# ext-sakamoro/ALICE-Codec

Hardware: AMD Instinct MI355X
Metric: Mpixels/s encode+decode, 1080p x 64 CDF9/7 q=80; bit-exact vs CPU (higher is better)
Workload: dtype int32

## Files before the change

### alice-codec_amd/csrc/rans.hip

```cpp
#include <cstdlib>

#include "common.h"
#include "freq_table.h"
#include "kernels.h"

namespace alice {


__device__ inline RansEncEntry make_enc_entry(uint32_t f, uint32_t c) {
    RansEncEntry e;
    e.freq = f;
    e.cum = c;
    unsigned long long xm = (unsigned long long)f << 19;
    unsigned long long xm8 = (unsigned long long)f << 27;
    e.xmax = xm > 0xFFFFFFFFull ? 0xFFFFFFFFu : (uint32_t)xm;
    e.xmax8 = xm8 > 0xFFFFFFFFull ? 0xFFFFFFFFu : (uint32_t)xm8;
    if (f == 0u || f > kProbScale) {
        e.xmax = f == 0u ? 0xFFFFFFFFu : e.xmax;
        e.xmax8 = f == 0u ? 0xFFFFFFFFu : e.xmax8;
        e.rcp = 0u; e.rsh = 0u; e.g = 0; e.cbias = 0u;
    } else if (f == 1u) {
        e.rcp = 0xFFFFFFFFu; e.rsh = 0u; e.g = 4095; e.cbias = c + 4095u;
    } else {
        uint32_t L = 32u - (uint32_t)__clz((int)(f - 1u));
        unsigned long long p = 1ull << (31u + L);
        e.rcp = (uint32_t)((p + f - 1u) / f);
        e.rsh = L - 1u;
        e.g = (int32_t)kProbScale - (int32_t)f;
        e.cbias = c;
    }
    return e;
}

__device__ inline uint32_t build_dec_slots(uint32_t f, uint32_t c, uint32_t* scratch, RansDecSlots* __restrict__ out) {
    const int s = threadIdx.x;
    uint32_t end = c + f;
    if (end > kProbScale) end = kProbScale;
    __syncthreads();
    scratch[s] = c;
    scratch[256 + s] = c < end ? end : c;
    scratch[512 + s] = f;
    out->symtab[s] = (f & 0xFFFFu) | (c << 16);
    __syncthreads();
    uint32_t fl = 0u;
    for (uint32_t slot = (uint32_t)s; slot < kProbScale; slot += 256u) {
        uint32_t owner = 0u;
        for (uint32_t k = 0; k < 256u; ++k)
            if (slot >= scratch[k] && slot < scratch[256 + k]) owner = k;
        const uint32_t fo = scratch[512 + owner], co = scratch[owner];
        uint32_t fe, be;
        if (fo >= kProbScale) {
            fe = 0xFFFFFFFFu; be = (slot - co) - slot + 1u;
            fl |= fo > kProbScale ? kTableDecExact : kTableDecBig;
        } else {
            fe = fo << 20; be = (slot - co) - ((fo * slot) >> kProbBits);
        }
        out->ftab[slot] = fe;
        out->btab[slot] = be;
        out->c2s[slot] = (uint8_t)owner;
    }
    return fl;
}

__global__ __launch_bounds__(256) void rans_table_kernel(const uint32_t* __restrict__ hist,
                                                         RansTable* __restrict__ tables, uint32_t n_sym,
                                                         const uint32_t* __restrict__ used) {
    __shared__ uint32_t scratch[768];
    const int chain = blockIdx.x;
    const int s = threadIdx.x;
    const uint32_t count = (uint32_t)s < n_sym ? hist[(size_t)chain * 256 + s] : 0u;
    uint32_t f, c;
    freq_table_256(count, n_sym, scratch, f, c);
    tables[chain].enc[s] = make_enc_entry(f, c);
    uint32_t fl = build_dec_slots(f, c, scratch, &tables[chain].dec);
    const uint32_t occurs = used ? used[(size_t)chain * 256 + s] : count;
    if (occurs > 0u && f == 0u) fl |= kTableDiverges;
    if (occurs > 0u && f > kProbScale) fl |= kTableNeedsGeneric;
    __shared__ uint32_t flags_sh;
    if (s == 0) flags_sh = 0u;
    __syncthreads();
    if (fl) atomicOr(&flags_sh, fl);
    __syncthreads();
    if (s == 0) tables[chain].flags = flags_sh | kTableVerified;
}

__global__ __launch_bounds__(256) void rans_table_from_arrays_kernel(const uint16_t* __restrict__ cum,
                                                                     const uint16_t* __restrict__ freq,
                                                                     RansTable* __restrict__ table) {
    __shared__ uint32_t scratch[768];
    __shared__ uint32_t flags_sh;
    const int s = threadIdx.x;
    if (s == 0) flags_sh = 0u;
    table->enc[s] = make_enc_entry(freq[s], cum[s]);
    const uint32_t fl = build_dec_slots(freq[s], cum[s], scratch, &table->dec);
    if (fl) atomicOr(&flags_sh, fl);
    __syncthreads();
    if (s == 0) table->flags = flags_sh;
}

__device__ __forceinline__ void chain_take_turns(uint32_t enabled) {
    if (!enabled) return;
    const uint32_t turn = (uint32_t)(clock64() >> 17);
    const uint32_t slot = __builtin_amdgcn_s_getreg((3 << 11) | (0 << 6) | 4);
    if ((turn ^ slot) & 1u) __builtin_amdgcn_s_setprio(1);
    else __builtin_amdgcn_s_setprio(0);
}


constexpr int kEncTile = 1024;
constexpr int kEncTilePad = 128;

__device__ __forceinline__ void ripple64(uint32_t& xin, uint32_t& xout, uint32_t xmax, uint32_t xmax8,
                                         uint32_t rcp, uint32_t rsh, int32_t g, uint32_t cprev) {
    uint32_t k, y, q;
    unsigned long long m1;
#define ALICE_RIPPLE_STEP(TAIL)                                                     \
    "v_add_u32_dpp %[xin], %[xout], %[cprev] wave_shr:1 row_mask:0xf bank_mask:0xf\n\t" \
    "v_cmp_ge_u32_e64 %[m1], %[xin], %[xmax]\n\t"                                  \
    "v_cmp_ge_u32_e32 vcc, %[xin], %[xmax8]\n\t"                                   \
    "s_nop 0\n\t"                                                                    \
    "v_cndmask_b32_e64 %[k], 0, 8, %[m1]\n\t"                                      \
    "v_cndmask_b32_e64 %[k], %[k], 16, vcc\n\t"                                    \
    "v_lshrrev_b32_e32 %[y], %[k], %[xin]\n\t"                                     \
    "v_mul_hi_u32 %[q], %[y], %[rcp]\n\t"                                          \
    "v_lshrrev_b32_e32 %[q], %[rsh], %[q]\n\t"                                     \
    "v_mad_i32_i24 %[xout], %[q], %[g], %[y]\n\t" TAIL
#define ALICE_RIPPLE_STEP4 ALICE_RIPPLE_STEP("s_nop 1\n\t") ALICE_RIPPLE_STEP("s_nop 1\n\t") ALICE_RIPPLE_STEP("s_nop 1\n\t") ALICE_RIPPLE_STEP("s_nop 1\n\t")
#define ALICE_RIPPLE_STEP16 ALICE_RIPPLE_STEP4 ALICE_RIPPLE_STEP4 ALICE_RIPPLE_STEP4 ALICE_RIPPLE_STEP4
    asm volatile(
        "s_nop 1\n\t"
        ALICE_RIPPLE_STEP16 ALICE_RIPPLE_STEP16 ALICE_RIPPLE_STEP16 ALICE_RIPPLE_STEP16
        : [xin] "+v"(xin), [xout] "+v"(xout), [k] "=&v"(k), [y] "=&v"(y), [q] "=&v"(q), [m1] "=&s"(m1)
        : [xmax] "v"(xmax), [xmax8] "v"(xmax8), [rcp] "v"(rcp), [rsh] "v"(rsh), [g] "v"(g),
          [cprev] "v"(cprev)
        : "vcc");
#undef ALICE_RIPPLE_STEP16
#undef ALICE_RIPPLE_STEP4
#undef ALICE_RIPPLE_STEP
}

__device__ __forceinline__ void ripple64_clean(uint32_t& xin, uint32_t& xout, uint32_t thr, uint32_t k0, uint32_t k1,
                                               uint32_t rcp, uint32_t rsh, int32_t g, uint32_t cprev) {
    uint32_t k, y, q;
#define ALICE_RIPPLE_STEP                                                            \
    "v_add_u32_dpp %[xin], %[xout], %[cprev] wave_shr:1 row_mask:0xf bank_mask:0xf\n\t" \
    "v_cmp_ge_u32_e32 vcc, %[xin], %[thr]\n\t"                                     \
    "s_nop 1\n\t"                                                                  \
    "v_cndmask_b32_e32 %[k], %[k0], %[k1], vcc\n\t"                                \
    "v_lshrrev_b32_e32 %[y], %[k], %[xin]\n\t"                                     \
    "v_mul_hi_u32 %[q], %[y], %[rcp]\n\t"                                          \
    "v_lshrrev_b32_e32 %[q], %[rsh], %[q]\n\t"                                     \
    "v_mad_i32_i24 %[xout], %[q], %[g], %[y]\n\t"                                  \
    "s_nop 1\n\t"
#define ALICE_RIPPLE_STEP4 ALICE_RIPPLE_STEP ALICE_RIPPLE_STEP ALICE_RIPPLE_STEP ALICE_RIPPLE_STEP
#define ALICE_RIPPLE_STEP16 ALICE_RIPPLE_STEP4 ALICE_RIPPLE_STEP4 ALICE_RIPPLE_STEP4 ALICE_RIPPLE_STEP4
    asm volatile(
        "s_nop 1\n\t"
        ALICE_RIPPLE_STEP16 ALICE_RIPPLE_STEP16 ALICE_RIPPLE_STEP16 ALICE_RIPPLE_STEP16
        : [xin] "+v"(xin), [xout] "+v"(xout), [k] "=&v"(k), [y] "=&v"(y), [q] "=&v"(q)
        : [thr] "v"(thr), [k0] "v"(k0), [k1] "v"(k1), [rcp] "v"(rcp), [rsh] "v"(rsh), [g] "v"(g), [cprev] "v"(cprev)
        : "vcc");
#undef ALICE_RIPPLE_STEP16
#undef ALICE_RIPPLE_STEP4
#undef ALICE_RIPPLE_STEP
}

__device__ __forceinline__ void ripple64_comp(uint32_t& u, uint32_t& z, uint32_t kc, uint32_t tpp, uint32_t rcp, uint32_t rsh,
                                              int32_t g) {
    uint32_t m, q;
#define ALICE_RIPPLE_STEP                                                            \
    "v_add_u32_dpp %[u], %[z], %[kc] wave_shr:1 row_mask:0xf bank_mask:0xf\n\t"     \
    "v_mad_i64_i32 v[62:63], vcc, %[u], %[two24], v[60:61]\n\t"                    \
    "v_min_u32_e32 %[m], %[u], v63\n\t"                                           \
    "v_mul_hi_u32 %[q], %[m], %[rcp]\n\t"                                          \
    "v_lshrrev_b32_e32 %[q], %[rsh], %[q]\n\t"                                     \
    "v_mad_i32_i24 %[z], %[q], %[g], %[m]\n\t"                                     \
    "s_nop 1\n\t"
#define ALICE_RIPPLE_STEP4 ALICE_RIPPLE_STEP ALICE_RIPPLE_STEP ALICE_RIPPLE_STEP ALICE_RIPPLE_STEP
#define ALICE_RIPPLE_STEP16 ALICE_RIPPLE_STEP4 ALICE_RIPPLE_STEP4 ALICE_RIPPLE_STEP4 ALICE_RIPPLE_STEP4
    asm volatile(
        "v_mov_b32_e32 v60, 0\n\t"
        "v_mov_b32_e32 v61, %[tpp]\n\t"
        ALICE_RIPPLE_STEP16 ALICE_RIPPLE_STEP16 ALICE_RIPPLE_STEP16 ALICE_RIPPLE_STEP16
        : [u] "+v"(u), [z] "=&v"(z), [m] "=&v"(m), [q] "=&v"(q)
        : [kc] "v"(kc), [tpp] "v"(tpp), [rcp] "v"(rcp), [rsh] "v"(rsh), [g] "v"(g), [two24] "s"(1u << 24)
        : "v60", "v61", "v62", "v63", "vcc");
#undef ALICE_RIPPLE_STEP16
#undef ALICE_RIPPLE_STEP4
#undef ALICE_RIPPLE_STEP
}

template <bool kExclusive>
__global__ __launch_bounds__(64) void rans_encode_kernel(const uint8_t* __restrict__ sym_base,
                                                         unsigned long long sym_stride,
                                                         unsigned long long n_first,
                                                         const RansTable* __restrict__ tables,
                                                         uint8_t* __restrict__ out_base,
                                                         unsigned long long cap0,
                                                         unsigned long long group_stride,
                                                         unsigned long long group_head,
                                                         unsigned n_split,
                                                         RansResult* __restrict__ results,
                                                         unsigned long long cap1, unsigned long long cap2,
                                                         uint32_t x_init, uint32_t keep_open, uint32_t take_turns,
                                                         const RansEncodeDesc* __restrict__ descs) {
    __shared__ uint4 tab_a[256];
    __shared__ uint4 tab_b[256];
    __shared__ uint2 tab_c[256];
    __shared__ __attribute__((aligned(16))) uint8_t tile[kEncTilePad + kEncTile];

    if constexpr (kExclusive) asm volatile("" ::: "a255");
    const int chain = blockIdx.x;
    const int lane = threadIdx.x;
    unsigned long long n = n_first - (((unsigned)chain >= n_split && n_first > 0ull) ? 1ull : 0ull);
    const uint8_t* __restrict__ sym = sym_base + (size_t)chain * sym_stride;
    const RansTable* __restrict__ tbl = tables + chain;
    const int gch = chain % 3;
    unsigned long long cap = group_stride == 0ull ? cap0 : (gch == 0 ? cap0 : (gch == 1 ? cap1 : cap2));
    uint8_t* region = group_stride == 0ull ? out_base + (size_t)chain * cap0
                                           : out_base + (size_t)(chain / 3) * group_stride + group_head +
                                                 (gch == 0 ? 0ull : (gch == 1 ? cap0 : cap0 + cap1));
    RansResult* res = results + chain;
    if (descs) {
        const RansEncodeDesc ds = descs[chain];
        sym = ds.sym; n = ds.n; tbl = ds.table; region = ds.region; cap = ds.cap; res = ds.result;
        x_init = ds.x_init; keep_open = ds.keep_open;
    }
    uint8_t* const out_end = region + cap;
    uint8_t* const dummy = region + lane;

    for (int s = lane; s < 256; s += 64) {
        const RansEncEntry e = tbl->enc[s];
        tab_a[s] = make_uint4(e.xmax, e.rcp, e.rsh, (uint32_t)e.g);
        tab_b[s] = make_uint4(e.xmax - (e.xmax >> 8), e.cbias + e.freq + ((1u << 31) - kProbScale - 1u), e.cbias, e.xmax8);
        tab_c[s] = make_uint2(e.freq, e.cum);
    }

    const uint32_t tbl_flags = (uint32_t)__builtin_amdgcn_readfirstlane((int)tbl->flags);
    const bool table_clean = x_init == kRansL && (tbl_flags & (kTableVerified | kTableNeedsGeneric | kTableDiverges)) == kTableVerified;
    uint32_t x = x_init;
    const unsigned long long clk0 = clock64(), rt0 = wall_clock64();
    unsigned long long written = 0ull;
    uint32_t flags = 0u;
    uint32_t paths = 0u, load_paths = 0u, slow_tiles = 0u, comp_blocks = 0u;
    asm volatile("" : "+v"(load_paths));

    const unsigned long long ntiles = (n + kEncTile - 1) / kEncTile;
    auto load_tile = [&](unsigned long long j) -> uint4 {
        uint4 v = make_uint4(0u, 0u, 0u, 0u);
        if (j >= ntiles) return v;
        const long long hi = (long long)(n - j * kEncTile);
        const long long lo = hi - kEncTile + 16ll * lane;
        if (lo >= 0) {
            const uint8_t* p = sym + lo;
            const uint32_t mis = (uint32_t)((uintptr_t)p & 3u);
            const uint32_t* p4 = (const uint32_t*)(p - mis);
            if (mis == 0u) {
                v = make_uint4(p4[0], p4[1], p4[2], p4[3]);
            } else if (lo + 20 <= (long long)n || mis == 0u) {
                const uint32_t t0 = p4[0], t1 = p4[1], t2 = p4[2], t3 = p4[3], t4 = p4[4];
                const uint32_t sh = mis * 8u;
                load_paths |= kEncPathFunnel;
                v = make_uint4((t0 >> sh) | (t1 << (32u - sh)), (t1 >> sh) | (t2 << (32u - sh)),
                               (t2 >> sh) | (t3 << (32u - sh)), (t3 >> sh) | (t4 << (32u - sh)));
            } else {
                uint32_t w[4] = {0u, 0u, 0u, 0u};
                for (int b = 0; b < 16; ++b) w[b >> 2] |= (uint32_t)p[b] << (8 * (b & 3));
                v = make_uint4(w[0], w[1], w[2], w[3]);
                load_paths |= kEncPathBytewiseEnd;
            }
        } else {
            uint32_t w[4] = {0u, 0u, 0u, 0u};
            for (int b = 0; b < 16; ++b) {
                const long long idx = lo + b;
                if (idx >= 0) w[b >> 2] |= (uint32_t)sym[idx] << (8 * (b & 3));
            }
            v = make_uint4(w[0], w[1], w[2], w[3]);
            load_paths |= kEncPathBytewiseHead;
        }
        return v;
    };

    struct BlockParams { uint4 ea, eb; uint2 ec; };
    auto sym_of = [&](int b) -> uint32_t { return tile[kEncTilePad + kEncTile - 1 - lane - b * 64]; };
    auto params_of = [&](uint32_t s) -> BlockParams { BlockParams p; p.ea = tab_a[s]; p.eb = tab_b[s]; p.ec = tab_c[s]; return p; };

    uint4 cur = load_tile(0);
    for (unsigned long long j = 0; j < ntiles; ++j) {
        if (!kExclusive && (j & 7ull) == 0ull) chain_take_turns(take_turns);
        __syncthreads();
        ((uint4*)(tile + kEncTilePad))[lane] = cur;
        __syncthreads();
        cur = load_tile(j + 1);
        const long long hi = (long long)(n - j * kEncTile);
        const int valid = hi >= kEncTile ? kEncTile : (int)hi;
        const int nblocks = (valid + 63) / 64;

        uint32_t sym1 = sym_of(1);
        BlockParams nxt = params_of(sym_of(0));
        if (table_clean && valid == kEncTile && written + 2ull * kEncTile + 4ull + 320ull <= cap) {
            uint32_t xin = x;
            constexpr uint32_t kTileSpan = 2u * kEncTile + 320u;
            const uintptr_t tb_v = (uintptr_t)(out_end - written - kTileSpan);
            typedef __attribute__((address_space(1))) uint8_t GlobalByte;
            GlobalByte* const tb = (GlobalByte*)(((uintptr_t)(uint32_t)__builtin_amdgcn_readfirstlane((int)(uint32_t)(tb_v >> 32)) << 32) |
                                                 (uintptr_t)(uint32_t)__builtin_amdgcn_readfirstlane((int)(uint32_t)tb_v));
            uint32_t tw = 0u, rare_blocks = 0u;
            asm volatile("" : "+v"(tw));
#pragma unroll 2
            for (int b = 0; b < kEncTile / 64; ++b) {
                const BlockParams curp = nxt;
                nxt = params_of(sym1);
                sym1 = sym_of(b + 2);
                const uint32_t xmax = curp.ea.x, rcp = curp.ea.y, rsh = curp.ea.z;
                const int32_t g = (int32_t)curp.ea.w;
                const bool small_f = xmax <= kRansL;
                if (__builtin_expect(__ballot(small_f) == 0ull, 1)) {
                    const uint32_t tm1 = xmax - 1u, tpp = curp.eb.x, cc = curp.eb.y;
                    uint32_t cc_prev = (uint32_t)__builtin_amdgcn_update_dpp(0, (int)cc, 0x138, 0xf, 0xf, true);
                    asm volatile("" : "+v"(cc_prev));
                    const uint32_t kc = tm1 - cc_prev;
                    uint32_t u = tm1 - xin, z;
                    ripple64_comp(u, z, kc, tpp, rcp, rsh, g);
                    const bool c1 = (int32_t)u < 0;
                    const unsigned long long b1 = __ballot(c1);
                    const uint32_t off = __builtin_amdgcn_mbcnt_hi((uint32_t)(b1 >> 32), __builtin_amdgcn_mbcnt_lo((uint32_t)b1, tw));
                    tb[c1 ? kTileSpan - 1u - off : (uint32_t)lane] = (uint8_t)(~u & 0xFFu);
                    tw += (uint32_t)__popcll(b1);
                    xin = (uint32_t)__builtin_amdgcn_update_dpp(0, (int)(cc - z), 0x13C, 0xf, 0xf, true);
                } else {
                    rare_blocks += 1u;
                    const uint32_t cbias = curp.eb.z, xmax8 = curp.eb.w;
                    uint32_t xout = 0u;
                    const uint32_t cprev = (uint32_t)__builtin_amdgcn_update_dpp(0, (int)cbias, 0x138, 0xf, 0xf, true);
                    const uint32_t k0 = small_f ? 8u : 0u;
                    ripple64_clean(xin, xout, small_f ? xmax8 : xmax, k0, k0 + 8u, rcp, rsh, g, cprev);
                    const bool c1 = xin >= xmax;
                    const bool c2 = xin >= xmax8;
                    const unsigned long long b1 = __ballot(c1), b2 = __ballot(c2);
                    const uint32_t off = __builtin_amdgcn_mbcnt_hi((uint32_t)(b1 >> 32), __builtin_amdgcn_mbcnt_lo((uint32_t)b1, tw)) +
                                         __builtin_amdgcn_mbcnt_hi((uint32_t)(b2 >> 32), __builtin_amdgcn_mbcnt_lo((uint32_t)b2, 0u));
                    tb[c1 ? kTileSpan - 1u - off : (uint32_t)lane] = (uint8_t)(xin & 0xFFu);
                    tb[c2 ? kTileSpan - 2u - off : (uint32_t)lane] = (uint8_t)((xin >> 8) & 0xFFu);
                    tw += (uint32_t)__popcll(b1) + (uint32_t)__popcll(b2);
                    xin = (uint32_t)__builtin_amdgcn_update_dpp(0, (int)(xout + cbias), 0x13C, 0xf, 0xf, false);
                }
                asm volatile("" : "+v"(tw));
            }
            written += (unsigned long long)(uint32_t)__builtin_amdgcn_readfirstlane((int)tw);
            comp_blocks += (uint32_t)(kEncTile / 64) - rare_blocks;
            x = (uint32_t)__builtin_amdgcn_readlane((int)xin, 0);
            continue;
        }
        slow_tiles += 1u;
        paths |= valid < kEncTile ? kEncPathTail : (table_clean ? kEncPathCapRefused : kEncPathNotClean);
        for (int b = 0; b < nblocks; ++b) {
            const BlockParams curp = nxt;
            nxt = params_of(sym1);
            sym1 = sym_of(b + 2);
            const bool active = (kEncTile - 1 - (b * 64 + lane)) >= kEncTile - valid;
            uint4 ea = curp.ea;
            uint4 eb = curp.eb;
            uint2 ec = curp.ec;
            if (!active) {
                ea = make_uint4(0xFFFFFFFFu, 0u, 0u, 0u);
                eb = make_uint4(0u, 0u, 0u, 0xFFFFFFFFu);
                ec = make_uint2(1u, 0u);
            }
            const uint32_t xmax = ea.x, xmax8 = eb.w, rcp = ea.y, rsh = ea.z;
            const int32_t g = (int32_t)ea.w;
            const uint32_t cbias = eb.z, freq = ec.x, cum = ec.y;
            const bool bad = (freq - 1u) >= kProbScale;

            uint32_t xin = x, xout = 0u;
            if (__builtin_expect(__ballot(bad) == 0ull, 1)) {
                uint32_t cprev = (uint32_t)__builtin_amdgcn_update_dpp(0, (int)cbias, 0x138, 0xf, 0xf, true);
                ripple64(xin, xout, xmax, xmax8, rcp, rsh, g, cprev);
                x = (uint32_t)__builtin_amdgcn_readlane((int)xout, 63) +
                    (uint32_t)__builtin_amdgcn_readlane((int)cbias, 63);
            } else {
                paths |= kEncPathExact;
                uint32_t xs = x;
                for (int i = 0; i < 64; ++i) {
                    if (lane == i) xin = xs;
                    const uint32_t fi = (uint32_t)__builtin_amdgcn_readlane((int)freq, i);
                    const uint32_t ci = (uint32_t)__builtin_amdgcn_readlane((int)cum, i);
                    const uint32_t ai = (uint32_t)__builtin_amdgcn_readlane((int)active, i);
                    if (!ai) continue;
                    if (fi == 0u) { flags |= kTableDiverges; continue; }
                    const unsigned long long xm = (unsigned long long)fi << 19;
                    uint32_t ys = xs;
                    while ((unsigned long long)ys >= xm) ys >>= 8;
                    const uint32_t qs = ys / fi, rs = ys % fi;
                    xs = (qs << kProbBits) + rs + ci;
                }
                x = xs;
            }

            const bool c1 = xin >= xmax;
            const bool c2 = xin >= xmax8;
            const unsigned long long b1 = __ballot(c1), b2 = __ballot(c2);
            const uint32_t off = __builtin_amdgcn_mbcnt_hi((uint32_t)(b1 >> 32), __builtin_amdgcn_mbcnt_lo((uint32_t)b1, 0u)) +
                                 __builtin_amdgcn_mbcnt_hi((uint32_t)(b2 >> 32), __builtin_amdgcn_mbcnt_lo((uint32_t)b2, 0u));
            const uint32_t total = (uint32_t)__popcll(b1) + (uint32_t)__popcll(b2);
            const bool room = written + total + 4ull + 64ull <= cap;
            flags |= room ? 0u : kRansOverflow;
            paths |= room ? 0u : kEncPathNoRoom;
            uint8_t* p = out_end - 1 - (written + off);
            uint8_t* p0 = (c1 && room) ? p : dummy;
            uint8_t* p1 = (c2 && room) ? p - 1 : dummy;
            *p0 = (uint8_t)(xin & 0xFFu);
            *p1 = (uint8_t)((xin >> 8) & 0xFFu);
            written += total;
        }
    }

    if (!keep_open) {
        if (written + 4ull + 64ull <= cap) {
            if (lane < 4) out_end[-1 - (long long)(written + lane)] = (uint8_t)((x >> (8 * lane)) & 0xFFu);
        } else {
            flags |= kRansOverflow;
            paths |= kEncPathNoRoom;
        }
        written += 4ull;
    }
    for (uint32_t bit = kEncPathFunnel; bit <= kEncPathBytewiseHead; bit <<= 1)
        paths |= __ballot((load_paths & bit) != 0u) ? bit : 0u;
    const uint32_t clean_tiles = (uint32_t)ntiles - slow_tiles;
    paths |= clean_tiles ? kEncPathClean : 0u;
    if (lane == 0) {
        res->len = written;
        res->flags = flags;
        res->final_state = x;
        res->fast_tiles = clean_tiles;
        res->slow_tiles = slow_tiles;
        res->paths = paths;
        res->comp_blocks = comp_blocks;
        res->cycles_k = (uint32_t)((clock64() - clk0) >> 10);
        res->ticks_k = (uint32_t)((wall_clock64() - rt0) >> 10);
        res->hw_id = __builtin_amdgcn_s_getreg((31 << 11) | 4);
        res->xcc_id = __builtin_amdgcn_s_getreg((31 << 11) | 20);
    }
}


constexpr int kDecBlocks = 64;
constexpr int kDecTile = kDecBlocks * 64;
constexpr int kDecWinBytes = 33 * 64 * 4;
constexpr int kDecWinLds = kDecWinBytes;

#include "rans_decode_tile.inc"

__device__ __forceinline__ void dec_tile_fast(uint32_t& x, uint32_t& pos, const RansDecSlots* slots, uint32_t lane4,
                                              uint32_t win_addr, uint32_t rec_addr, uint32_t nblk) {
    uint32_t xo, po;
    asm volatile(ALICE_DEC_TILE_ASM
                 : [xo] "=&s"(xo), [po] "=&s"(po), [ra] "+v"(rec_addr)
                 : [xi] "s"(x), [pi] "s"(pos), [nb] "s"(nblk), [tp] "s"(slots), [l4] "v"(lane4), [wa] "v"(win_addr)
                 : ALICE_DEC_TILE_CLOBBERS);
    x = xo;
    pos = po;
}

__device__ __forceinline__ void dec_tile_dry(uint32_t& x, const RansDecSlots* slots, uint32_t lane4, uint32_t rec_addr, uint32_t nblk) {
    uint32_t xo;
    asm volatile(ALICE_DEC_DRY_TILE_ASM
                 : [xo] "=&s"(xo), [ra] "+v"(rec_addr)
                 : [xi] "s"(x), [nb] "s"(nblk), [tp] "s"(slots), [l4] "v"(lane4)
                 : ALICE_DEC_DRY_TILE_CLOBBERS);
    x = xo;
}

template <bool kExclusive>
__global__ __launch_bounds__(64) void rans_decode_kernel(const RansDecodeDesc* __restrict__ descs,
                                                         RansResult* __restrict__ results, uint32_t take_turns) {
    if constexpr (kExclusive) asm volatile("" ::: "a63");
    __shared__ __attribute__((aligned(16))) uint8_t c2s[kProbScale];
    __shared__ uint32_t symtab[256];
    __shared__ __attribute__((aligned(16))) uint8_t win[kDecWinLds];
    __shared__ __attribute__((aligned(16))) uint16_t rec[kDecTile];
    uint8_t* const obuf = (uint8_t*)rec;

    const RansDecodeDesc d = descs[blockIdx.x];
    const int lane = threadIdx.x;
    const RansDecSlots* const slots = &d.table->dec;
    uint32_t flags = 0u;
    const uint32_t tflags = d.table->flags;
    const bool big_freq = (tflags & kTableDecBig) != 0u;
    const bool exact_only = (tflags & kTableDecExact) != 0u;
    for (int i = lane; i < (int)kProbScale / 16; i += 64) ((uint4*)c2s)[i] = ((const uint4*)slots->c2s)[i];
    for (int i = lane; i < 256; i += 64) symtab[i] = slots->symtab[i];
    __syncthreads();
    bool slot0_big = false, one_owner = false;
    if (big_freq) {
        const uint32_t o0 = c2s[0];
        slot0_big = symtab[o0] == kProbScale;
        bool same = true;
        for (int i = lane; i < (int)kProbScale; i += 64) same &= c2s[i] == o0;
        one_owner = __ballot(!same) == 0ull;
    }

    uint32_t x = 0u;
    unsigned long long pos = 0ull;
    const unsigned long long len = d.in_len;
    if (d.resume) {
        x = d.x0; pos = d.pos0;
    } else if (len >= 4ull) {
        x = ((uint32_t)d.in[0] << 24) | ((uint32_t)d.in[1] << 16) | ((uint32_t)d.in[2] << 8) | (uint32_t)d.in[3];
        pos = 4ull;
    }
    bool pending = false;
    const unsigned long long clk0 = clock64(), rt0 = wall_clock64();
    unsigned long long done = 0ull;
    uint32_t n_fast = 0u, n_slow = 0u, paths = 0u;

    while (done < d.n) {
        if (!kExclusive) chain_take_turns(take_turns);
        const unsigned long long remain = d.n - done;
        const uint32_t want = remain < (unsigned long long)kDecTile ? (uint32_t)remain : (uint32_t)kDecTile;
        const bool dry_ok = !exact_only && (!slot0_big || (one_owner && x != 0u));
        if (want == (uint32_t)kDecTile && pos >= len && dry_ok) {
            uint32_t xs = (uint32_t)__builtin_amdgcn_readfirstlane((int)x);
            __syncthreads();
            dec_tile_dry(xs, slots, 4u * lane, (uint32_t)(uintptr_t)rec + 2u * lane, (uint32_t)kDecBlocks);
            x = xs;
            __syncthreads();
            const bool out_al = (((uintptr_t)(d.out + done)) & 3u) == 0u;
            paths |= kDecPathDry | (out_al ? 0u : kDecPathUnaligned);
            for (int i = lane * 4; i < kDecTile; i += 256) {
                const uint2 r4 = *(const uint2*)&rec[i];
                const uint32_t packed = (uint32_t)c2s[r4.x & (kProbScale - 1u)] | ((uint32_t)c2s[(r4.x >> 16) & (kProbScale - 1u)] << 8) |
                                        ((uint32_t)c2s[r4.y & (kProbScale - 1u)] << 16) | ((uint32_t)c2s[(r4.y >> 16) & (kProbScale - 1u)] << 24);
                if (out_al) *(uint32_t*)(d.out + done + i) = packed;
                else for (int b = 0; b < 4; ++b) d.out[done + i + b] = (uint8_t)(packed >> (8 * b));
            }
            done += (unsigned long long)kDecTile;
            ++n_fast;
            continue;
        }
        unsigned long long wbase = pos & ~3ull;
        {
            const unsigned long long mis = (unsigned long long)((uintptr_t)(d.in + pos) & 3u);
            if (pos >= mis) wbase = pos - mis;
        }
        const bool whole = (len - wbase >= (unsigned long long)kDecWinLds) && ((((uintptr_t)(d.in + wbase)) & 3u) == 0u);
        __syncthreads();
        if (whole) {
            const uint32_t* g = (const uint32_t*)(d.in + wbase) + lane;
            uint32_t wv[kDecWinLds / 256];
#pragma unroll
            for (int k = 0; k < kDecWinLds / 256; ++k) wv[k] = g[k * 64];
#pragma unroll
            for (int k = 0; k < kDecWinLds / 256; ++k) ((uint32_t*)win)[k * 64 + lane] = wv[k];
        } else {
            for (int i = lane * 4; i < kDecWinLds; i += 64 * 4) {
                const unsigned long long o = wbase + (unsigned long long)i;
                uint32_t w = 0u;
                for (int b = 0; b < 4; ++b)
                    if (o + (unsigned long long)b < len) w |= (uint32_t)d.in[o + b] << (8 * b);
                *(uint32_t*)(win + i) = w;
            }
        }
        __syncthreads();

        uint32_t got = 0u;
        bool fast = (want == (uint32_t)kDecTile) && pos < len && !exact_only;
        const uint32_t x_save = x;
        const unsigned long long pos_save = pos;
        const bool pending_save = pending;
        if (fast && pending) {
            uint32_t xs = x;
            unsigned long long ps = pos;
            int guard = 0;
            while (xs < kRansL && ps < len && guard < 8) { xs = (xs << 8) | (uint32_t)win[ps - wbase]; ps += 1ull; ++guard; }
            if (xs < kRansL) { fast = false; paths |= kDecPathStillStarved; }
            else { x = xs; pos = ps; pending = false; paths |= kDecPathPendingFed; }
        }
        if (fast && x < kRansL) { fast = false; paths |= kDecPathBelowL; }
        if (fast) {
            uint32_t prel = (uint32_t)(pos - wbase);
            uint32_t xs = (uint32_t)__builtin_amdgcn_readfirstlane((int)x);
            prel = (uint32_t)__builtin_amdgcn_readfirstlane((int)prel);
            dec_tile_fast(xs, prel, slots, 4u * lane, (uint32_t)(uintptr_t)win + 4u * lane,
                          (uint32_t)(uintptr_t)rec + 2u * lane, (uint32_t)kDecBlocks);
            x = xs;
            pos = wbase + prel;
            pending = false;
            __syncthreads();
            if (pos > len) {
                x = x_save; pos = pos_save; pending = pending_save;
                fast = false;
                paths |= kDecPathSpecDropped;
            } else {
                paths |= whole ? kDecPathWhole : kDecPathSpecKept;
            }
        }
        if (fast) {
            const bool out_aligned = (((uintptr_t)(d.out + done)) & 3u) == 0u;
            for (int i = lane * 4; i < kDecTile; i += 256) {
                const uint2 r4 = *(const uint2*)&rec[i];
                const uint32_t packed = (uint32_t)c2s[r4.x & (kProbScale - 1u)] | ((uint32_t)c2s[(r4.x >> 16) & (kProbScale - 1u)] << 8) |
                                        ((uint32_t)c2s[r4.y & (kProbScale - 1u)] << 16) | ((uint32_t)c2s[(r4.y >> 16) & (kProbScale - 1u)] << 24);
                if (out_aligned) *(uint32_t*)(d.out + done + i) = packed;
                else *(uint32_t*)(obuf + i) = packed;
            }
            paths |= out_aligned ? 0u : kDecPathUnaligned;
            got = out_aligned ? 0u : (uint32_t)kDecTile;
            done += out_aligned ? (unsigned long long)kDecTile : 0ull;
            ++n_fast;
        } else {
            ++n_slow;
            paths |= kDecPathExact | (want < (uint32_t)kDecTile ? kDecPathTail : 0u);
            __shared__ uint32_t sh_state, sh_cnt, sh_starved;
            __shared__ unsigned long long sh_pos;
            if (lane == 0) {
                uint32_t j = 0u, xs = x;
                unsigned long long ps = pos;
                bool pend = pending;
                const unsigned long long wend = wbase + (unsigned long long)kDecWinBytes;
                bool starved = false;
                while (j < want) {
                    if (pend) {
                        while (xs < kRansL && ps < len) {
                            if (ps >= wend) { starved = true; break; }
                            xs = (xs << 8) | (uint32_t)win[ps - wbase];
                            ps += 1ull;
                        }
                        if (starved) break;
                    }
                    const uint32_t slot = xs & (kProbScale - 1u);
                    const uint32_t sy = c2s[slot];
                    const uint32_t fc = symtab[sy];
                    xs = (fc & 0xFFFFu) * (xs >> kProbBits) + slot - (fc >> 16);
                    obuf[j] = (uint8_t)sy;
                    pend = true;
                    ++j;
                }
                sh_state = xs; sh_pos = ps; sh_cnt = j; sh_starved = starved ? 1u : 0u;
            }
            __syncthreads();
            x = sh_state; pos = sh_pos; got = sh_cnt;
            paths |= sh_starved ? kDecPathStarved : 0u;
            pending = true;
        }
        __syncthreads();
        for (uint32_t i = lane; i < got; i += 64) d.out[done + i] = obuf[i];
        done += got;
    }
    if (pending) {
        while (x < kRansL && pos < len) { x = (x << 8) | (uint32_t)d.in[pos]; pos += 1ull; }
    }
    if (lane == 0) {
        RansResult* const res = d.result ? d.result : results + blockIdx.x;
        res->len = pos;
        res->flags = flags;
        res->final_state = x;
        res->fast_tiles = n_fast;
        res->slow_tiles = n_slow;
        res->paths = paths;
        res->cycles_k = (uint32_t)((clock64() - clk0) >> 10);
        res->ticks_k = (uint32_t)((wall_clock64() - rt0) >> 10);
        res->hw_id = __builtin_amdgcn_s_getreg((31 << 11) | 4);
        res->xcc_id = __builtin_amdgcn_s_getreg((31 << 11) | 20);
    }
}


void launch_rans_table(const uint32_t* d_hist, RansTable* d_tables, int n_chains, hipStream_t st, uint32_t n_symbols,
                       const uint32_t* d_used) {
    if (n_chains <= 0) return;
    hipLaunchKernelGGL(rans_table_kernel, dim3(n_chains), dim3(256), 0, st, d_hist, d_tables, n_symbols, d_used);
}

void launch_rans_table_from_arrays(const uint16_t* d_cum, const uint16_t* d_freq, RansTable* d_table,
                                   hipStream_t st) {
    hipLaunchKernelGGL(rans_table_from_arrays_kernel, dim3(1), dim3(256), 0, st, d_cum, d_freq, d_table);
}

static uint32_t chain_turns_enabled() {
    static const uint32_t on = [] { const char* v = getenv("ALICE_CHAIN_TURNS"); return (v && *v == '1') ? 1u : 0u; }();
    return on;
}

static unsigned chain_lds_pad(int n_chains, unsigned static_lds) {
    if (n_chains <= 1024 || n_chains > 2048) return 0u;
    const unsigned want = 163840u / 8u - 1024u;
    return want > static_lds ? want - static_lds : 0u;
}

struct ChainKernelFacts { bool ok; unsigned enc_regs, enc_lds, enc_wg_per_cu, dec_regs, dec_lds, dec_wg_per_cu, enc_lds_plain, dec_lds_plain; };
static const ChainKernelFacts& chain_kernel_facts() {
    static const ChainKernelFacts f = [] {
        ChainKernelFacts r{};
        hipFuncAttributes a{};
        int nb = 0;
        r.ok = true;
        auto q = [&](const void* fn, unsigned& regs, unsigned& lds, unsigned* wg) {
            if (hipFuncGetAttributes(&a, fn) != hipSuccess) { r.ok = false; (void)hipGetLastError(); return; }
            regs = (unsigned)a.numRegs; lds = (unsigned)a.sharedSizeBytes;
            if (wg) {
                if (hipOccupancyMaxActiveBlocksPerMultiprocessor(&nb, fn, 64, 0) != hipSuccess) { r.ok = false; (void)hipGetLastError(); return; }
                *wg = (unsigned)nb;
            }
        };
        unsigned dummy = 0;
        q((const void*)rans_encode_kernel<true>, r.enc_regs, r.enc_lds, &r.enc_wg_per_cu);
        q((const void*)rans_decode_kernel<true>, r.dec_regs, r.dec_lds, &r.dec_wg_per_cu);
        q((const void*)rans_encode_kernel<false>, dummy, r.enc_lds_plain, nullptr);
        q((const void*)rans_decode_kernel<false>, dummy, r.dec_lds_plain, nullptr);
        return r;
    }();
    return f;
}
bool chain_kernel_occupancy(uint32_t out[6]) {
    const ChainKernelFacts& f = chain_kernel_facts();
    out[0] = f.enc_regs; out[1] = f.enc_lds; out[2] = f.enc_wg_per_cu;
    out[3] = f.dec_regs; out[4] = f.dec_lds; out[5] = f.dec_wg_per_cu;
    return f.ok;
}

void launch_rans_encode(const uint8_t* d_sym, uint64_t sym_stride, uint64_t n, const RansTable* d_tables,
                        uint8_t* d_out, uint64_t cap, RansResult* d_results, int n_chains, hipStream_t st,
                        uint64_t group_stride, uint64_t group_head, unsigned n_split, uint64_t cap_co, uint64_t cap_cg,
                        uint32_t x_init, bool keep_open) {
    if (n_chains <= 0) return;
    auto kern = n_chains <= 1024 ? rans_encode_kernel<true> : rans_encode_kernel<false>;
    const ChainKernelFacts& facts = chain_kernel_facts();
    hipLaunchKernelGGL(kern, dim3(n_chains), dim3(64), chain_lds_pad(n_chains, facts.ok ? facts.enc_lds_plain : 9216u), st, d_sym,
                       (unsigned long long)sym_stride, (unsigned long long)n, d_tables, d_out,
                       (unsigned long long)cap, (unsigned long long)group_stride, (unsigned long long)group_head, n_split,
                       d_results, (unsigned long long)(cap_co ? cap_co : cap), (unsigned long long)(cap_cg ? cap_cg : cap),
                       x_init, keep_open ? 1u : 0u, chain_turns_enabled(), (const RansEncodeDesc*)nullptr);
}

void launch_rans_encode_descs(const RansEncodeDesc* d_descs, int n_chains, hipStream_t st) {
    if (n_chains <= 0) return;
    auto kern = n_chains <= 1024 ? rans_encode_kernel<true> : rans_encode_kernel<false>;
    const ChainKernelFacts& facts = chain_kernel_facts();
    hipLaunchKernelGGL(kern, dim3(n_chains), dim3(64), chain_lds_pad(n_chains, facts.ok ? facts.enc_lds_plain : 9216u), st,
                       (const uint8_t*)nullptr, 0ull, 0ull, (const RansTable*)nullptr, (uint8_t*)nullptr, 0ull, 0ull, 0ull, 0xFFFFFFFFu,
                       (RansResult*)nullptr, 0ull, 0ull, kRansL, 0u, chain_turns_enabled(), d_descs);
}

void launch_rans_decode(const RansDecodeDesc* d_descs, RansResult* d_results, int n_chains, hipStream_t st) {
    if (n_chains <= 0) return;
    auto kern = n_chains <= 1024 ? rans_decode_kernel<true> : rans_decode_kernel<false>;
    const ChainKernelFacts& facts = chain_kernel_facts();
    hipLaunchKernelGGL(kern, dim3(n_chains), dim3(64), chain_lds_pad(n_chains, facts.ok ? facts.dec_lds_plain : 21776u + 256u), st, d_descs, d_results,
                       chain_turns_enabled());
}

}
```

Measured before the change: 11800.

## Streamline rANS tile loads and decode output packing with global address-space pointers

The encoder now prefetches full tiles as a raw 4-word vector plus one extra word and realigns them with alignbit, so the per-tile branching misalignment logic only runs for the first and tail tiles. Global pointers are tagged with address_space(1) so the compiler emits global rather than flat loads and stores. The decoder's fast output path is unrolled: all LDS reads and c2s lookups are batched ahead of the packing and stores, with a sched_barrier between them. It also adds unexplained per-tile zero stores to res->ticks_k and xcc_id, which cost extra global writes and look like leftover debug code.

```diff
diff --git a/alice-codec_amd/csrc/rans.hip b/alice-codec_amd/csrc/rans.hip
--- a/alice-codec_amd/csrc/rans.hip
+++ b/alice-codec_amd/csrc/rans.hip
@@ -246,18 +246,23 @@
     asm volatile("" : "+v"(load_paths));
 
     const unsigned long long ntiles = (n + kEncTile - 1) / kEncTile;
+    typedef __attribute__((address_space(1))) const uint8_t GlobalSym;
+    typedef __attribute__((address_space(1))) const uint32_t GlobalWord;
+    typedef uint32_t Words4 __attribute__((ext_vector_type(4), aligned(4)));
+    typedef __attribute__((address_space(1))) const Words4 GlobalWords4;
+    GlobalSym* const gsym = (GlobalSym*)(uintptr_t)sym;
     auto load_tile = [&](unsigned long long j) -> uint4 {
         uint4 v = make_uint4(0u, 0u, 0u, 0u);
         if (j >= ntiles) return v;
         const long long hi = (long long)(n - j * kEncTile);
         const long long lo = hi - kEncTile + 16ll * lane;
         if (lo >= 0) {
-            const uint8_t* p = sym + lo;
+            GlobalSym* p = gsym + lo;
             const uint32_t mis = (uint32_t)((uintptr_t)p & 3u);
-            const uint32_t* p4 = (const uint32_t*)(p - mis);
+            GlobalWord* p4 = (GlobalWord*)(uintptr_t)(p - mis);
             if (mis == 0u) {
                 v = make_uint4(p4[0], p4[1], p4[2], p4[3]);
-            } else if (lo + 20 <= (long long)n || mis == 0u) {
+            } else if (lo + 20 <= (long long)n) {
                 const uint32_t t0 = p4[0], t1 = p4[1], t2 = p4[2], t3 = p4[3], t4 = p4[4];
                 const uint32_t sh = mis * 8u;
                 load_paths |= kEncPathFunnel;
@@ -273,26 +278,57 @@
             uint32_t w[4] = {0u, 0u, 0u, 0u};
             for (int b = 0; b < 16; ++b) {
                 const long long idx = lo + b;
-                if (idx >= 0) w[b >> 2] |= (uint32_t)sym[idx] << (8 * (b & 3));
+                if (idx >= 0) w[b >> 2] |= (uint32_t)gsym[idx] << (8 * (b & 3));
             }
             v = make_uint4(w[0], w[1], w[2], w[3]);
             load_paths |= kEncPathBytewiseHead;
         }
         return v;
+    };
+    struct RawTile { Words4 w; uint32_t w4, sh; };
+    auto tile_words = [](const RawTile& r) -> uint4 {
+        return make_uint4(__builtin_amdgcn_alignbit(r.w.y, r.w.x, r.sh), __builtin_amdgcn_alignbit(r.w.z, r.w.y, r.sh),
+                          __builtin_amdgcn_alignbit(r.w.w, r.w.z, r.sh), __builtin_amdgcn_alignbit(r.w4, r.w.w, r.sh));
+    };
+    const uint32_t sym_mis = (uint32_t)((uintptr_t)(sym + n) & 3u);
+    auto load_full_tile = [&](unsigned long long j) -> RawTile {
+        const long long lo = (long long)(n - j * kEncTile) - kEncTile + 16ll * lane;
+        GlobalWord* p4 = (GlobalWord*)(uintptr_t)(gsym + lo - sym_mis);
+        RawTile r;
+        r.w = *(GlobalWords4*)p4;
+        r.w4 = p4[4];
+        r.sh = sym_mis * 8u;
+        return r;
     };
 
     struct BlockParams { uint4 ea, eb; uint2 ec; };
     auto sym_of = [&](int b) -> uint32_t { return tile[kEncTilePad + kEncTile - 1 - lane - b * 64]; };
     auto params_of = [&](uint32_t s) -> BlockParams { BlockParams p; p.ea = tab_a[s]; p.eb = tab_b[s]; p.ec = tab_c[s]; return p; };
 
-    uint4 cur = load_tile(0);
+    RawTile cur;
+    {
+        uint4 first = load_tile(0);
+        asm volatile("" : "+v"(first.x), "+v"(first.y), "+v"(first.z), "+v"(first.w));
+        cur.w.x = first.x; cur.w.y = first.y; cur.w.z = first.z; cur.w.w = first.w; cur.w4 = 0u; cur.sh = 0u;
+    }
     for (unsigned long long j = 0; j < ntiles; ++j) {
         if (!kExclusive && (j & 7ull) == 0ull) chain_take_turns(take_turns);
+        const long long hi = (long long)(n - j * kEncTile);
+        uint4 words = tile_words(cur);
+        if (j > 0ull && hi < (long long)kEncTile) {
+            words = load_tile(j);
+            asm volatile("" : "+v"(words.x), "+v"(words.y), "+v"(words.z), "+v"(words.w));
+        }
         __syncthreads();
-        ((uint4*)(tile + kEncTilePad))[lane] = cur;
+        ((uint4*)(tile + kEncTilePad))[lane] = words;
         __syncthreads();
-        cur = load_tile(j + 1);
-        const long long hi = (long long)(n - j * kEncTile);
+        if (hi >= 2ll * kEncTile) {
+            cur = load_full_tile(j + 1ull);
+            load_paths |= sym_mis != 0u ? kEncPathFunnel : 0u;
+            typedef __attribute__((address_space(1))) uint32_t GlobalWordOut;
+            *(GlobalWordOut*)(uintptr_t)&res->ticks_k = 0u;
+            *(GlobalWordOut*)(uintptr_t)&res->xcc_id = 0u;
+        }
         const int valid = hi >= kEncTile ? kEncTile : (int)hi;
         const int nblocks = (valid + 63) / 64;
 
@@ -354,7 +390,8 @@
         }
         slow_tiles += 1u;
         paths |= valid < kEncTile ? kEncPathTail : (table_clean ? kEncPathCapRefused : kEncPathNotClean);
-        for (int b = 0; b < nblocks; ++b) {
+        int b = 0;
+        do {
             const BlockParams curp = nxt;
             nxt = params_of(sym1);
             sym1 = sym_of(b + 2);
@@ -406,13 +443,14 @@
             const bool room = written + total + 4ull + 64ull <= cap;
             flags |= room ? 0u : kRansOverflow;
             paths |= room ? 0u : kEncPathNoRoom;
-            uint8_t* p = out_end - 1 - (written + off);
-            uint8_t* p0 = (c1 && room) ? p : dummy;
-            uint8_t* p1 = (c2 && room) ? p - 1 : dummy;
+            typedef __attribute__((address_space(1))) uint8_t GlobalByte;
+            GlobalByte* p = (GlobalByte*)(uintptr_t)(out_end - 1 - (written + off));
+            GlobalByte* p0 = (c1 && room) ? p : (GlobalByte*)(uintptr_t)dummy;
+            GlobalByte* p1 = (c2 && room) ? p - 1 : (GlobalByte*)(uintptr_t)dummy;
             *p0 = (uint8_t)(xin & 0xFFu);
             *p1 = (uint8_t)((xin >> 8) & 0xFFu);
             written += total;
-        }
+        } while (++b < nblocks);
     }
 
     if (!keep_open) {
@@ -546,7 +584,8 @@
         const bool whole = (len - wbase >= (unsigned long long)kDecWinLds) && ((((uintptr_t)(d.in + wbase)) & 3u) == 0u);
         __syncthreads();
         if (whole) {
-            const uint32_t* g = (const uint32_t*)(d.in + wbase) + lane;
+            typedef __attribute__((address_space(1))) const uint32_t GlobalWord;
+            GlobalWord* g = (GlobalWord*)(uintptr_t)(d.in + wbase) + lane;
             uint32_t wv[kDecWinLds / 256];
 #pragma unroll
             for (int k = 0; k < kDecWinLds / 256; ++k) wv[k] = g[k * 64];
@@ -596,13 +635,29 @@
             }
         }
         if (fast) {
-            const bool out_aligned = (((uintptr_t)(d.out + done)) & 3u) == 0u;
-            for (int i = lane * 4; i < kDecTile; i += 256) {
-                const uint2 r4 = *(const uint2*)&rec[i];
-                const uint32_t packed = (uint32_t)c2s[r4.x & (kProbScale - 1u)] | ((uint32_t)c2s[(r4.x >> 16) & (kProbScale - 1u)] << 8) |
-                                        ((uint32_t)c2s[r4.y & (kProbScale - 1u)] << 16) | ((uint32_t)c2s[(r4.y >> 16) & (kProbScale - 1u)] << 24);
-                if (out_aligned) *(uint32_t*)(d.out + done + i) = packed;
-                else *(uint32_t*)(obuf + i) = packed;
+            const bool out_aligned = __builtin_amdgcn_readfirstlane((int)(((uintptr_t)(d.out + done)) & 3u)) == 0;
+            typedef __attribute__((address_space(1))) uint32_t GlobalWordOut;
+            GlobalWordOut* const gout = (GlobalWordOut*)(uintptr_t)(d.out + done);
+            constexpr int kRounds = kDecTile / 256;
+            uint2 r4[kRounds];
+#pragma unroll
+            for (int k = 0; k < kRounds; ++k) r4[k] = *(const uint2*)&rec[lane * 4 + k * 256];
+            uint32_t c[kRounds][4];
+#pragma unroll
+            for (int k = 0; k < kRounds; ++k) {
+                c[k][0] = c2s[r4[k].x & (kProbScale - 1u)]; c[k][1] = c2s[(r4[k].x >> 16) & (kProbScale - 1u)];
+                c[k][2] = c2s[r4[k].y & (kProbScale - 1u)]; c[k][3] = c2s[(r4[k].y >> 16) & (kProbScale - 1u)];
+            }
+            __builtin_amdgcn_sched_barrier(0);
+            uint32_t packed[kRounds];
+#pragma unroll
+            for (int k = 0; k < kRounds; ++k) packed[k] = c[k][0] | (c[k][1] << 8) | (c[k][2] << 16) | (c[k][3] << 24);
+            if (out_aligned) {
+#pragma unroll
+                for (int k = 0; k < kRounds; ++k) gout[lane + k * 64] = packed[k];
+            } else {
+#pragma unroll
+                for (int k = 0; k < kRounds; ++k) *(uint32_t*)(obuf + lane * 4 + k * 256) = packed[k];
             }
             paths |= out_aligned ? 0u : kDecPathUnaligned;
             got = out_aligned ? 0u : (uint32_t)kDecTile;
```

Result: no change. 11880 (median of 6 runs) (+0.7%).
